# iPieter/llmq

Hardware: AMD Instinct MI355X
Metric: output_tokens_per_sec (Tower-Plus-9B continuous-batching serving decode) (higher is better)
Workload: dtype bf16; 1 GPU; model=tower-plus-9b (gemma-2-9b arch, random init), global_batch=512, seq_len=1024, parallelism=dp1, kv_cache_dtype=auto

## Files before the change

### llmq_amd/engine/model_runner.py

```python

from __future__ import annotations

import logging
import time
from typing import Dict, List, Optional, Tuple

import numpy as np
import torch

from llmq_amd import ops
from llmq_amd.engine.config import EngineConfig
from llmq_amd.engine.forward_meta import ChunkGather, DecodeMeta, MixedMeta, PrefillMeta
from llmq_amd.engine.kv_cache import KVCache
from llmq_amd.engine.models.llama import CausalLM
from llmq_amd.engine.scheduler import ScheduledBatch, Sequence

logger = logging.getLogger(__name__)


def _buckets(max_bs: int) -> List[int]:
    sizes = [1, 2, 4, 8, 16, 24, 32, 48, 64, 96, 128, 192, 256, 384, 512]
    out = [b for b in sizes if b < max_bs]
    out.append(max_bs)
    return out


class ModelRunner:
    def __init__(
        self,
        model: CausalLM,
        kv_cache: KVCache,
        config: EngineConfig,
        device: torch.device,
        max_model_len: int,
    ):
        self.model = model
        self.kv_cache = kv_cache
        self.config = config
        self.device = device
        self.max_model_len = max_model_len
        self.block_size = kv_cache.block_size
        self.max_blocks_per_seq = (max_model_len + self.block_size - 1) // self.block_size
        self.use_graphs = (
            config.enable_hipgraph
            and not config.enforce_eager
            and device.type == "cuda"
        )
        self._graphs: Dict[int, torch.cuda.CUDAGraph] = {}
        self._graph_pool = None
        self.sampling_generator = torch.Generator(device=device if device.type == "cuda" else "cpu")
        self.sampling_generator.manual_seed(config.seed)
        self._sample_step = 0
        self._sample_bufs: Dict[str, Dict[str, torch.Tensor]] = {}
        if self.use_graphs:
            self._alloc_static_buffers()


    def _alloc_static_buffers(self) -> None:
        B = min(self.config.max_num_seqs, self.config.hipgraph_max_batch)
        dev = self.device
        self.graph_max_bs = B
        self.in_ids = torch.zeros(B, dtype=torch.long, device=dev)
        self.in_pos = torch.zeros(B, dtype=torch.long, device=dev)
        self.in_slots = torch.zeros(B, dtype=torch.long, device=dev)
        self.in_block_tables = torch.zeros(
            B, self.max_blocks_per_seq, dtype=torch.int32, device=dev
        )
        self.in_context_lens = torch.ones(B, dtype=torch.int32, device=dev)
        self.out_hidden = torch.zeros(
            B, self.model.spec.hidden_size, dtype=self.model.dtype, device=dev
        )
        self.h_ids = torch.zeros(B, dtype=torch.long, pin_memory=True)
        self.h_pos = torch.zeros(B, dtype=torch.long, pin_memory=True)
        self.h_slots = torch.zeros(B, dtype=torch.long, pin_memory=True)
        self.h_block_tables = torch.zeros(
            B, self.max_blocks_per_seq, dtype=torch.int32, pin_memory=True
        )
        self.h_context_lens = torch.ones(B, dtype=torch.int32, pin_memory=True)
        self._staged_rows: List[Tuple[int, int, int]] = [(-1, -1, 0)] * B

    def capture_graphs(self) -> None:
        if not self.use_graphs:
            return
        t0 = time.perf_counter()
        torch.cuda.synchronize()
        for bs in reversed(_buckets(self.graph_max_bs)):
            meta = DecodeMeta(
                block_tables=self.in_block_tables[:bs],
                context_lens=self.in_context_lens[:bs],
                slot_mapping=self.in_slots[:bs],
            )
            out = self.model.forward(self.in_ids[:bs], self.in_pos[:bs], self.kv_cache, meta)
            torch.cuda.synchronize()
            graph = torch.cuda.CUDAGraph()
            with torch.cuda.graph(graph, pool=self._graph_pool):
                out = self.model.forward(
                    self.in_ids[:bs], self.in_pos[:bs], self.kv_cache, meta
                )
                self.out_hidden[:bs].copy_(out)
            if self._graph_pool is None:
                self._graph_pool = graph.pool()
            self._graphs[bs] = graph
        torch.cuda.synchronize()
        logger.info(
            "captured %d decode hipGraphs (max_bs=%d) in %.1fs",
            len(self._graphs), self.graph_max_bs, time.perf_counter() - t0,
# ... 22 lines not shown
        krow = 0
        for seq, (start, end) in zip(pseqs, chunks):
            n = end - start
            ids.extend(seq.token_ids[start:end])
            pos.extend(range(start, end))
            bt = seq.block_table
            slots.extend(bt[p // bs] * bs + (p % bs) for p in range(start, end))
            if end == seq.num_tokens:
                rel_last.append(cu[-1] + n - 1)
            cu.append(cu[-1] + n)
            if any_chunk:
                for p in range(start):
                    g_blocks.append(bt[p // bs])
                    g_offs.append(p % bs)
                    past_dst.append(krow)
                    krow += 1
                for i in range(cu[-2], cu[-1]):
                    fresh_dst.append(krow)
                    krow += 1
            cu_k.append(cu_k[-1] + end)
        slot_mapping = torch.tensor(slots, dtype=torch.long, device=dev)
        gather = None
        if any_chunk:
            gather = ChunkGather(
                cu_seqlens_k=torch.tensor(cu_k, dtype=torch.int32, device=dev),
                blocks=torch.tensor(g_blocks, dtype=torch.long, device=dev),
                offs=torch.tensor(g_offs, dtype=torch.long, device=dev),
                past_dst=torch.tensor(past_dst, dtype=torch.long, device=dev),
                fresh_dst=torch.tensor(fresh_dst, dtype=torch.long, device=dev),
                total_k=krow,
            )
        meta = PrefillMeta(
            cu_seqlens=torch.tensor(cu, dtype=torch.int32, device=dev),
            max_seqlen=max(e - st for (st, e) in chunks),
            slot_mapping=slot_mapping,
            gather=gather,
        )
        return ids, pos, slot_mapping, meta, rel_last

    @torch.no_grad()
    def execute_prefill(self, seqs: List[Sequence], chunks=None, buf_name: str = "main") -> torch.Tensor:
        if chunks is None:
            chunks = [(0, s.num_tokens) for s in seqs]
        dev = self.device
        ids, pos, slot_mapping, meta, rel_last = self._build_prefill_meta(
            seqs, chunks, dev
        )
        input_ids = torch.tensor(ids, dtype=torch.long, device=dev)
        positions = torch.tensor(pos, dtype=torch.long, device=dev)
        hidden = self.model.forward(input_ids, positions, self.kv_cache, meta)
        if not rel_last:
            return torch.empty(0, dtype=torch.long, device=dev)
        last_hidden = hidden[torch.tensor(rel_last, dtype=torch.long, device=dev)]
        logits = self.model.compute_logits(last_hidden)
        sample_seqs = [s for s, (st, e) in zip(seqs, chunks) if e == s.num_tokens]
        return self._sample(logits, sample_seqs, buf_name)


    @torch.no_grad()
    def execute_mixed(self, batch: "ScheduledBatch") -> torch.Tensor:
        dev = self.device
        dseqs = batch.seqs[: batch.n_decode]
        pseqs = batch.seqs[batch.n_decode :]
        chunks = batch.chunks or [(0, s.num_tokens) for s in pseqs]
        bs = self.block_size
        nd = len(dseqs)

        ids = [s.token_ids[-1] for s in dseqs]
        pos = [s.num_tokens - 1 for s in dseqs]
        slots = [s.block_table[p // bs] * bs + (p % bs) for s, p in zip(dseqs, pos)]
        ctx = [s.num_tokens for s in dseqs]
        p_ids, p_pos, p_slots, pmeta, rel_last = self._build_prefill_meta(
            pseqs, chunks, dev
        )
        ids.extend(p_ids)
        pos.extend(p_pos)

        block_tables = torch.zeros(
            nd, max(len(s.block_table) for s in dseqs), dtype=torch.int32, device=dev
        )
        bt_np = np.zeros(tuple(block_tables.shape), dtype=np.int32)
        for i, s in enumerate(dseqs):
            bt_np[i, : len(s.block_table)] = s.block_table
        block_tables.copy_(torch.from_numpy(bt_np))
        d_slots = torch.tensor(slots, dtype=torch.long, device=dev)
        slot_mapping = torch.cat([d_slots, p_slots])
        meta = MixedMeta(
            n_decode=nd,
            decode=DecodeMeta(
                block_tables=block_tables,
                context_lens=torch.tensor(ctx, dtype=torch.int32, device=dev),
                slot_mapping=d_slots,
            ),
            prefill=pmeta,
            slot_mapping=slot_mapping,
        )
        input_ids = torch.tensor(ids, dtype=torch.long, device=dev)
        positions = torch.tensor(pos, dtype=torch.long, device=dev)
        hidden = self.model.forward(input_ids, positions, self.kv_cache, meta)
        last_idx = list(range(nd)) + [nd + r for r in rel_last]
        last_hidden = hidden[torch.tensor(last_idx, dtype=torch.long, device=dev)]
        logits = self.model.compute_logits(last_hidden)
        sample_seqs = list(dseqs) + [
            s for s, (st, e) in zip(pseqs, chunks) if e == s.num_tokens
        ]
        return self._sample(logits, sample_seqs)


    @torch.no_grad()
    def execute_decode(self, seqs: List[Sequence], force_eager: bool = False) -> torch.Tensor:
        dev = self.device
        B = len(seqs)
        bs = self.block_size
        ids = [s.token_ids[-1] for s in seqs]
        pos = [s.num_tokens - 1 for s in seqs]
        slots = [s.block_table[p // bs] * bs + (p % bs) for s, p in zip(seqs, pos)]
        ctx = [s.num_tokens for s in seqs]

        bucket = self._bucket_for(B) if (self.use_graphs and not force_eager) else None
        if bucket is not None and bucket in self._graphs:
            return self._decode_with_graph(seqs, bucket, ids, pos, slots, ctx)

        block_tables = torch.zeros(
            B, max(len(s.block_table) for s in seqs), dtype=torch.int32, device=dev
        )
        bt_np = np.zeros(tuple(block_tables.shape), dtype=np.int32)
        for i, s in enumerate(seqs):
            bt_np[i, : len(s.block_table)] = s.block_table
        block_tables.copy_(torch.from_numpy(bt_np))
        meta = DecodeMeta(
            block_tables=block_tables,
            context_lens=torch.tensor(ctx, dtype=torch.int32, device=dev),
            slot_mapping=torch.tensor(slots, dtype=torch.long, device=dev),
        )
        input_ids = torch.tensor(ids, dtype=torch.long, device=dev)
        positions = torch.tensor(pos, dtype=torch.long, device=dev)
        hidden = self.model.forward(input_ids, positions, self.kv_cache, meta)
        logits = self.model.compute_logits(hidden)
        return self._sample(logits, seqs)

    def _decode_with_graph(
        self, seqs: List[Sequence], bucket: int, ids, pos, slots, ctx
    ) -> torch.Tensor:
        B = len(seqs)
        self.h_ids[:B] = torch.tensor(ids, dtype=torch.long)
        self.h_pos[:B] = torch.tensor(pos, dtype=torch.long)
        self.h_slots[:B] = torch.tensor(slots, dtype=torch.long)
        self.h_context_lens[:B] = torch.tensor(ctx, dtype=torch.int32)
        self.h_context_lens[B:bucket] = 1
        bt_np = self.h_block_tables.numpy()
        max_w = 1
        for i, s in enumerate(seqs):
            n = len(s.block_table)
            if n > max_w:
                max_w = n
            if self._staged_rows[i] != (s.uid, s.num_preemptions, n):
                bt_np[i, :n] = s.block_table
                self._staged_rows[i] = (s.uid, s.num_preemptions, n)
        if B < bucket:
            self.h_slots[B:bucket] = 0
            self.h_ids[B:bucket] = 0
            self.h_pos[B:bucket] = 0
            for i in range(B, bucket):
                if self._staged_rows[i] != (-1, -1, 0):
                    bt_np[i, :1] = 0
                    self._staged_rows[i] = (-1, -1, 0)
        self.in_ids[:bucket].copy_(self.h_ids[:bucket], non_blocking=True)
        self.in_pos[:bucket].copy_(self.h_pos[:bucket], non_blocking=True)
        self.in_slots[:bucket].copy_(self.h_slots[:bucket], non_blocking=True)
        self.in_context_lens[:bucket].copy_(self.h_context_lens[:bucket], non_blocking=True)
        self.in_block_tables[:bucket, :max_w].copy_(
            self.h_block_tables[:bucket, :max_w], non_blocking=True
        )
        self._graphs[bucket].replay()
        logits = self.model.compute_logits(self.out_hidden[:B])
        return self._sample(logits, seqs)


    def _sample_buf(self, name: str, B: int, dev) -> Dict[str, torch.Tensor]:
        buf = self._sample_bufs.get(name)
        if buf is None or buf["out"].numel() < B:
            cap = max(B, self.config.max_num_seqs)
            buf = {
                "out": torch.empty(cap, dtype=torch.int64, device=dev),
                "keys": torch.empty(cap, dtype=torch.int64, device=dev),
                "temps": torch.empty(cap, dtype=torch.float32, device=dev),
                "temps_h": torch.empty(cap, dtype=torch.float32, pin_memory=True),
                "seeds": torch.empty(cap, dtype=torch.int32, device=dev),
                "seeds_h": torch.empty(cap, dtype=torch.int32, pin_memory=True),
                "pos": torch.empty(cap, dtype=torch.int32, device=dev),
                "pos_h": torch.empty(cap, dtype=torch.int32, pin_memory=True),
            }
            self._sample_bufs[name] = buf
        return buf

    def _sample(self, logits: torch.Tensor, seqs: List[Sequence],
                buf_name: str = "main") -> torch.Tensor:
        dev = logits.device
        self._sample_step += 1
        simple = all(
            s.params.top_k == 0 and s.params.top_p >= 1.0 for s in seqs
        )
        if dev.type == "cuda":
            B = len(seqs)
            buf = self._sample_buf(buf_name, B, dev)
            th = buf["temps_h"]
            sh = buf["seeds_h"]
            ph = buf["pos_h"]
            for i, s in enumerate(seqs):
                th[i] = s.params.temperature
                rs = s.params.seed
                if rs is None:
                    sh[i] = 0
                else:
                    v = rs & 0x7FFFFFFF
                    sh[i] = v if v else 0x1E3779B9
                ph[i] = s.output_len
            buf["temps"][:B].copy_(th[:B], non_blocking=True)
            buf["seeds"][:B].copy_(sh[:B], non_blocking=True)
            buf["pos"][:B].copy_(ph[:B], non_blocking=True)
            logits_f = logits.float()
            bounds = None
            if not simple:
                tps = torch.tensor([s.params.top_p for s in seqs],
                                   dtype=torch.float32, device=dev)
                tks = torch.tensor([s.params.top_k for s in seqs],
                                   dtype=torch.int64, device=dev)
                bounds = ops.topk_topp_bound(
                    logits_f, buf["temps"][:B], tps, tks)
            ops.sample_gumbel_argmax(
                buf["out"][:B], buf["keys"][:B], logits_f,
                buf["temps"][:B], buf["seeds"][:B],
                buf["pos"][:B], self.config.seed, self._sample_step, bounds,
            )
            return buf["out"][:B]
        temps = torch.tensor([s.params.temperature for s in seqs], dtype=torch.float32, device=dev)
        tps = torch.tensor([s.params.top_p for s in seqs], dtype=torch.float32, device=dev)
        tks = torch.tensor([s.params.top_k for s in seqs], dtype=torch.int64, device=dev)
        out = ops.sample_tokens(logits, temps, tps, tks, self.sampling_generator)
        seeded = [
            i for i, s in enumerate(seqs)
            if s.params.seed is not None and s.params.temperature > 0
        ]
        if seeded:
            idx = torch.tensor(seeded, dtype=torch.long, device=dev)
            rows = logits[idx].float().cpu()
            temps_c, tps_c, tks_c = temps[idx].cpu(), tps[idx].cpu(), tks[idx].cpu()
            redraw = torch.empty(len(seeded), dtype=out.dtype)
            for j, i in enumerate(seeded):
                s = seqs[i]
                g = torch.Generator(device="cpu")
                g.manual_seed((s.params.seed << 20) ^ s.output_len)
                redraw[j] = ops.sample_tokens(
                    rows[j : j + 1], temps_c[j : j + 1], tps_c[j : j + 1],
                    tks_c[j : j + 1], g,
                )[0]
            out[idx] = redraw.to(out.device)
        return out
```

### llmq_amd/engine/models/llama.py

```python

from __future__ import annotations

import math
import os
from typing import Dict, List, Optional, Union

import torch
import torch.nn.functional as F

from llmq_amd import ops
from llmq_amd.engine.forward_meta import DecodeMeta, MixedMeta, PrefillMeta
from llmq_amd.engine.kv_cache import KVCache
from llmq_amd.engine.model_specs import ModelSpec
from llmq_amd.parallel import get_tp_group


_USE_SKINNY_GEMM = os.environ.get("LLMQ_SKINNY_GEMM", "0") not in ("0", "false", "")


def _proj(x: torch.Tensor, w: torch.Tensor, bias=None) -> torch.Tensor:
    if (_USE_SKINNY_GEMM and x.is_cuda and x.dtype == torch.bfloat16
            and x.shape[0] <= 1024 and w.shape[1] % 64 == 0
            and w.shape[0] % 4 == 0):
        return ops.skinny_gemm(x, w, bias)
# ... 198 lines not shown
                self.rope_cache, meta.slot_mapping,
            )
            window = s.sliding_window if s.layer_uses_sliding_window(i) else 0
            if meta.is_prefill:
                attn = self._prefill_attn(q, k, v, meta, kv_cache, i, window)
            elif meta.is_mixed:
                nd = meta.n_decode
                attn_d = ops.paged_decode_attention(
                    q[:nd], kv_cache.k[i], kv_cache.v[i],
                    meta.decode.block_tables, meta.decode.context_lens,
                    s.scale, s.attn_softcap, window,
                )
                attn_p = self._prefill_attn(
                    q[nd:], k[nd:], v[nd:], meta.prefill, kv_cache, i, window
                )
                attn = torch.cat([attn_d, attn_p], dim=0)
            else:
                attn = ops.paged_decode_attention(
                    q, kv_cache.k[i], kv_cache.v[i], meta.block_tables,
                    meta.context_lens, s.scale, s.attn_softcap, window,
                )
            attn_out = _proj(attn.reshape(T, self.q_size), lw.o)
            if tp is not None:
                attn_out = tp.all_reduce(attn_out)
            if s.post_norms:
                h, residual = ops.norm_add_norm(
                    attn_out, residual, lw.post_attn_norm, lw.pre_mlp_norm,
                    s.rms_eps, self.norm_offset,
                )
            else:
                h, residual = ops.fused_add_rmsnorm(
                    attn_out, residual, lw.pre_mlp_norm, s.rms_eps, self.norm_offset
                )
            gate_up = _proj(h, lw.gate_up)
            act = ops.gelu_tanh_and_mul(gate_up) if s.gelu else ops.silu_and_mul(gate_up)
            mlp_out = _proj(act, lw.down)
            if tp is not None:
                mlp_out = tp.all_reduce(mlp_out)
            w_next = (
                self.layers[i + 1].input_norm if i + 1 < n_layers else self.final_norm
            )
            if s.post_norms:
                h, residual = ops.norm_add_norm(
                    mlp_out, residual, lw.post_mlp_norm, w_next,
                    s.rms_eps, self.norm_offset,
                )
            else:
                h, residual = ops.fused_add_rmsnorm(
                    mlp_out, residual, w_next, s.rms_eps, self.norm_offset
                )
        return h

    @torch.no_grad()
    def compute_logits(self, hidden: torch.Tensor) -> torch.Tensor:
        logits = _proj(hidden, self.lm_head).float()
        cap = self.spec.final_softcap
        if cap and cap > 0:
            logits = torch.tanh(logits / cap) * cap
        return logits
```

### llmq_amd/ops/__init__.py

```python

from __future__ import annotations

import os
from pathlib import Path
from typing import Optional, Tuple

import torch

from llmq_amd.ops import torch_ref

_EXT = None
_EXT_ERROR: Optional[str] = None
_EXT_TRIED = False


def _try_load_extension() -> None:
    global _EXT, _EXT_ERROR, _EXT_TRIED
    if _EXT_TRIED:
        return
    _EXT_TRIED = True
    here = Path(__file__).parent
    override = os.environ.get("LLMQ_OPS_SO")
    if override:
        candidates = [Path(override)]
# ... 154 lines not shown
    cu_seqlens: torch.Tensor,
    max_seqlen: int,
    scale: float,
    softcap: float = 0.0,
    window: int = 0,
    cu_seqlens_k: Optional[torch.Tensor] = None,
) -> torch.Tensor:
    cu_k = cu_seqlens if cu_seqlens_k is None else cu_seqlens_k
    if _use_hip(q):
        out = torch.empty_like(q)
        _EXT.varlen_prefill_attention(
            out, q, k, v, cu_seqlens, cu_k, int(max_seqlen), scale, softcap, window
        )
        return out
    return torch_ref.varlen_prefill_attention(
        q, k, v, cu_seqlens, scale, softcap, window, cu_seqlens_k=cu_k
    )




def skinny_gemm(
    x: torch.Tensor,
    w: torch.Tensor,
    bias: Optional[torch.Tensor] = None,
    splitk: int = 0,
    out: Optional[torch.Tensor] = None,
) -> torch.Tensor:
    M, K = x.shape
    N = w.shape[0]
    if not (x.is_cuda and x.dtype == torch.bfloat16 and K % 64 == 0
            and N % 4 == 0 and has_hip_ext()):
        import torch.nn.functional as F

        return F.linear(x, w, bias)
    if out is None:
        out = torch.empty(M, N, dtype=torch.bfloat16, device=x.device)
    _EXT.skinny_gemm(out, x, w, bias, splitk)
    return out




def sample_gumbel_argmax(
    out: torch.Tensor,
    keys: torch.Tensor,
    logits: torch.Tensor,
    temps: torch.Tensor,
    req_seeds: torch.Tensor,
    req_pos: torch.Tensor,
    seed: int,
    step: int,
    bounds: Optional[torch.Tensor] = None,
) -> None:
    assert _use_hip(logits)
    keys.zero_()
    _EXT.sample_gumbel_argmax(out, keys, logits, temps, req_seeds, req_pos,
                              seed, step, bounds)


def topk_topp_bound(
    logits: torch.Tensor,
    temps: torch.Tensor,
    top_ps: torch.Tensor,
    top_ks: torch.Tensor,
) -> torch.Tensor:
    assert _use_hip(logits)
    out = torch.empty(logits.size(0), dtype=torch.float32, device=logits.device)
    _EXT.topk_topp_bound(out, logits, temps, top_ps, top_ks)
    return out


def sample_tokens(
    logits: torch.Tensor,
    temperatures: torch.Tensor,
    top_ps: torch.Tensor,
    top_ks: torch.Tensor,
    generator: Optional[torch.Generator] = None,
) -> torch.Tensor:
    if logits.is_cuda:
        return _sample_tokens_gpu(logits, temperatures, top_ps, top_ks, generator)
    return torch_ref.sample_tokens(logits, temperatures, top_ps, top_ks, generator)


def _sample_tokens_gpu(
    logits: torch.Tensor,
    temperatures: torch.Tensor,
    top_ps: torch.Tensor,
    top_ks: torch.Tensor,
    generator: Optional[torch.Generator],
) -> torch.Tensor:
    B, V = logits.shape
    greedy = temperatures <= 0
    temps = torch.where(greedy, torch.ones_like(temperatures), temperatures)
    scaled = logits.float() / temps.unsqueeze(1)
    need_topk = bool((top_ks > 0).any()) and bool((top_ks < V).any())
    need_topp = bool((top_ps < 1.0).any())
    if need_topk or need_topp:
        bound = topk_topp_bound(logits.float(), temperatures.float(),
                                top_ps.float(), top_ks)
        scaled = torch.where(logits.float() >= bound.unsqueeze(1), scaled,
                             torch.full_like(scaled, float("-inf")))
    u = torch.rand(B, V, device=logits.device, generator=generator)
    gumbel = -torch.log(-torch.log(u.clamp_min(1e-20)).clamp_min(1e-20))
    sampled = (scaled + gumbel).argmax(dim=-1)
    greedy_choice = logits.argmax(dim=-1)
    return torch.where(greedy, greedy_choice, sampled)
```

### llmq_amd/ops/hip/bindings.cpp

```cpp

#include <ATen/ATen.h>
#include <c10/hip/HIPStream.h>
#include <hip/hip_runtime.h>
#include <torch/library.h>

#include <hip/hip_bf16.h>
#include <hip/hip_fp16.h>


namespace {

#define CHECK_GPU(x) TORCH_CHECK(x.is_cuda(), #x " must be on GPU")
#define CHECK_LASTDIM(x) \
  TORCH_CHECK(x.stride(-1) == 1, #x " innermost dim must be contiguous")

hipStream_t stream() { return c10::hip::getCurrentHIPStream().stream(); }

template <typename F>
void dispatch_dtype(const at::Tensor& t, const char* name, F&& f) {
  switch (t.scalar_type()) {
    case at::kBFloat16:
      f.template operator()<__hip_bfloat16>();
      break;
    case at::kHalf:
// ... 54 lines not shown
                       reinterpret_cast<T*>(residual.data_ptr()),
                       reinterpret_cast<const T*>(weight.data_ptr()), hidden,
                       (float)eps, (float)offset);
  });
}


template <bool GELU>
void act_and_mul(at::Tensor out, at::Tensor in) {
  CHECK_GPU(in);
  CHECK_LASTDIM(in);
  const int d = out.size(-1);
  const long rows = out.numel() / d;
  TORCH_CHECK(in.size(-1) == 2 * d, "in must be [..., 2*d]");
  const long chunks = rows * (d / 8);
  const int grid = std::min<long>((chunks + 255) / 256, 2048);
  dispatch_dtype(in, "act_and_mul", [&]<typename T>() {
    hipLaunchKernelGGL((act_and_mul_kernel<T, GELU>), dim3(grid), dim3(256), 0,
                       stream(), reinterpret_cast<T*>(out.data_ptr()),
                       reinterpret_cast<const T*>(in.data_ptr()), rows, d);
  });
}

void silu_and_mul(at::Tensor out, at::Tensor in) { act_and_mul<false>(out, in); }
void gelu_tanh_and_mul(at::Tensor out, at::Tensor in) { act_and_mul<true>(out, in); }


void rope_inplace(at::Tensor q, at::Tensor k, at::Tensor positions,
                  at::Tensor cos_sin) {
  CHECK_GPU(q);
  CHECK_LASTDIM(q);
  CHECK_LASTDIM(k);
  TORCH_CHECK(q.dim() == 3 && k.dim() == 3, "q/k must be [T, H, D]");
  TORCH_CHECK(cos_sin.scalar_type() == at::kFloat, "cos_sin must be f32");
  const int T_ = q.size(0);
  if (T_ == 0) return;
  const int hq = q.size(1), hk = k.size(1), d = q.size(2);
  TORCH_CHECK(q.stride(1) == d && k.stride(1) == d, "head dim must be packed");
  dispatch_dtype(q, "rope", [&]<typename T>() {
    hipLaunchKernelGGL(rope_kernel<T>, dim3(T_), dim3(256), 0, stream(),
                       reinterpret_cast<T*>(q.data_ptr()),
                       reinterpret_cast<T*>(k.data_ptr()),
                       positions.data_ptr<long>(), cos_sin.data_ptr<float>(),
                       hq, hk, d, q.stride(0), k.stride(0));
  });
}

void norm_add_norm(at::Tensor x, at::Tensor residual, at::Tensor w_post,
                   at::Tensor w_pre, double eps, double offset) {
  CHECK_GPU(x);
  CHECK_LASTDIM(x);
  const int hidden = x.size(-1);
  const long rows = x.numel() / hidden;
  dispatch_dtype(x, "norm_add_norm", [&]<typename T>() {
    hipLaunchKernelGGL(norm_add_norm_kernel<T>, dim3(rows), dim3(256), 0,
                       stream(), reinterpret_cast<T*>(x.data_ptr()),
                       reinterpret_cast<T*>(residual.data_ptr()),
                       reinterpret_cast<const T*>(w_post.data_ptr()),
                       reinterpret_cast<const T*>(w_pre.data_ptr()), hidden,
                       (float)eps, (float)offset);
  });
}


void reshape_and_cache(at::Tensor key, at::Tensor value, at::Tensor k_cache,
                       at::Tensor v_cache, at::Tensor slot_mapping) {
  CHECK_GPU(key);
  CHECK_LASTDIM(key);
  const int T_ = key.size(0);
  if (T_ == 0) return;
  const int kvh = key.size(1), d = key.size(2);
  const int bs = k_cache.size(2);
  TORCH_CHECK(k_cache.is_contiguous() && v_cache.is_contiguous());
  TORCH_CHECK(slot_mapping.scalar_type() == at::kLong);
  const bool fp8_cache = k_cache.scalar_type() == at::kFloat8_e4m3fn;
  dispatch_dtype(key, "reshape_and_cache", [&]<typename T>() {
    dispatch_cache_type<T>(fp8_cache, [&]<typename TC>() {
      hipLaunchKernelGGL((reshape_and_cache_kernel<T, TC>), dim3(T_), dim3(128),
                         0, stream(), reinterpret_cast<const T*>(key.data_ptr()),
                         reinterpret_cast<const T*>(value.data_ptr()),
                         reinterpret_cast<TC*>(k_cache.data_ptr()),
                         reinterpret_cast<TC*>(v_cache.data_ptr()),
                         slot_mapping.data_ptr<long>(), kvh, d, bs,
                         key.stride(0), value.stride(0));
    });
  });
}

void rope_and_cache(at::Tensor q, at::Tensor k, at::Tensor value,
                    at::Tensor k_cache, at::Tensor v_cache,
                    at::Tensor positions, at::Tensor cos_sin,
                    at::Tensor slot_mapping) {
  CHECK_GPU(q);
  CHECK_LASTDIM(q);
  CHECK_LASTDIM(k);
  TORCH_CHECK(q.dim() == 3 && k.dim() == 3, "q/k must be [T, H, D]");
  TORCH_CHECK(cos_sin.scalar_type() == at::kFloat);
  TORCH_CHECK(slot_mapping.scalar_type() == at::kLong);
  const int T_ = q.size(0);
  if (T_ == 0) return;
  const int hq = q.size(1), hk = k.size(1), d = q.size(2);
  const int bs = k_cache.size(2);
  TORCH_CHECK(q.stride(1) == d && k.stride(1) == d, "head dim must be packed");
  const bool fp8_cache = k_cache.scalar_type() == at::kFloat8_e4m3fn;
  dispatch_dtype(q, "rope_and_cache", [&]<typename T>() {
    dispatch_cache_type<T>(fp8_cache, [&]<typename TC>() {
      hipLaunchKernelGGL((rope_and_cache_kernel<T, TC>), dim3(T_), dim3(256), 0,
                         stream(), reinterpret_cast<T*>(q.data_ptr()),
                         reinterpret_cast<T*>(k.data_ptr()),
                         reinterpret_cast<const T*>(value.data_ptr()),
                         reinterpret_cast<TC*>(k_cache.data_ptr()),
                         reinterpret_cast<TC*>(v_cache.data_ptr()),
                         positions.data_ptr<long>(), cos_sin.data_ptr<float>(),
// ... 189 lines not shown
  TORCH_CHECK(out.scalar_type() == at::kBFloat16 && out.is_contiguous());
  const int M = x.size(0), K = x.size(1), N = w.size(0);
  TORCH_CHECK(w.size(1) == K && out.size(0) == M && out.size(1) == N);
  TORCH_CHECK(K % SKG_BK == 0, "K must be a multiple of 64");
  TORCH_CHECK(N % 4 == 0, "N must be a multiple of 4");
  const __hip_bfloat16* bias_ptr = nullptr;
  if (bias.has_value() && bias->defined()) {
    TORCH_CHECK(bias->scalar_type() == at::kBFloat16 && bias->numel() == N);
    bias_ptr = reinterpret_cast<const __hip_bfloat16*>(bias->data_ptr());
  }
  const int mt = (M + SKG_BM - 1) / SKG_BM;
  const int nt = (N + SKG_BN - 1) / SKG_BN;
  int z = (int)splitk;
  if (z <= 0) {
    z = 1;
    while (mt * nt * z < 256 && (K / SKG_BK) / (z * 2) >= 8 && z < 8) z *= 2;
  }
  dim3 grid(mt, nt, z);
  static const int sync_dbg = [] {
    const char* e = getenv("LLMQ_SKG_SYNC");
    return e ? atoi(e) : 0;
  }();
  if (z == 1) {
    if (sync_dbg) {
      hipLaunchKernelGGL((skinny_gemm_kernel<0, 1>), grid, dim3(SKG_NT), 0,
                         stream(), out.data_ptr(),
                         reinterpret_cast<const __hip_bfloat16*>(x.data_ptr()),
                         reinterpret_cast<const __hip_bfloat16*>(w.data_ptr()),
                         bias_ptr, M, N, K, x.stride(0), w.stride(0));
      return;
    }
    hipLaunchKernelGGL((skinny_gemm_kernel<0>), grid, dim3(SKG_NT), 0, stream(),
                       out.data_ptr(),
                       reinterpret_cast<const __hip_bfloat16*>(x.data_ptr()),
                       reinterpret_cast<const __hip_bfloat16*>(w.data_ptr()),
                       bias_ptr, M, N, K, x.stride(0), w.stride(0));
    return;
  }
  at::Tensor slabs = at::empty({z, (long)M * N}, x.options().dtype(at::kFloat));
  hipLaunchKernelGGL((skinny_gemm_kernel<1>), grid, dim3(SKG_NT), 0, stream(),
                     slabs.data_ptr(),
                     reinterpret_cast<const __hip_bfloat16*>(x.data_ptr()),
                     reinterpret_cast<const __hip_bfloat16*>(w.data_ptr()),
                     nullptr, M, N, K, x.stride(0), w.stride(0));
  const long MN = (long)M * N;
  const long blocks = (MN / 4 + 255) / 256;
  hipLaunchKernelGGL(skinny_gemm_reduce_kernel, dim3(blocks), dim3(256), 0,
                     stream(),
                     reinterpret_cast<__hip_bfloat16*>(out.data_ptr()),
                     slabs.data_ptr<float>(), bias_ptr, z, MN, N);
}


void topk_topp_bound(at::Tensor out_bound, at::Tensor logits, at::Tensor temps,
                     at::Tensor top_ps, at::Tensor top_ks) {
  CHECK_GPU(logits);
  TORCH_CHECK(logits.scalar_type() == at::kFloat && logits.dim() == 2);
  TORCH_CHECK(out_bound.scalar_type() == at::kFloat);
  TORCH_CHECK(top_ps.scalar_type() == at::kFloat);
  TORCH_CHECK(top_ks.scalar_type() == at::kLong);
  const int B = logits.size(0), V = logits.size(1);
  hipLaunchKernelGGL(topk_topp_bound_kernel, dim3(B), dim3(256), 0, stream(),
                     out_bound.data_ptr<float>(), logits.data_ptr<float>(),
                     temps.data_ptr<float>(), top_ps.data_ptr<float>(),
                     top_ks.data_ptr<long>(), V, logits.stride(0));
}

void sample_gumbel_argmax(at::Tensor out, at::Tensor keys, at::Tensor logits,
                          at::Tensor temps, at::Tensor req_seeds,
                          at::Tensor req_pos, long seed, long step,
                          c10::optional<at::Tensor> bounds) {
  CHECK_GPU(logits);
  TORCH_CHECK(logits.scalar_type() == at::kFloat && logits.dim() == 2);
  TORCH_CHECK(out.scalar_type() == at::kLong);
  TORCH_CHECK(keys.scalar_type() == at::kLong && keys.numel() == logits.size(0));
  TORCH_CHECK(req_seeds.scalar_type() == at::kInt);
  TORCH_CHECK(req_pos.scalar_type() == at::kInt);
  const int B = logits.size(0), V = logits.size(1);
  const float* bounds_ptr = nullptr;
  if (bounds.has_value() && bounds->defined()) {
    TORCH_CHECK(bounds->scalar_type() == at::kFloat && bounds->numel() == B);
    bounds_ptr = bounds->data_ptr<float>();
  }
  int nsplit = 1;
  while (B * nsplit < 2048 && nsplit < 64 && (V / nsplit) > 4096) nsplit *= 2;
  hipLaunchKernelGGL(sample_argmax_kernel, dim3(B, nsplit), dim3(256), 0,
                     stream(),
                     reinterpret_cast<unsigned long long*>(keys.data_ptr()),
                     logits.data_ptr<float>(), temps.data_ptr<float>(),
                     reinterpret_cast<const unsigned int*>(req_seeds.data_ptr()),
                     reinterpret_cast<const unsigned int*>(req_pos.data_ptr()),
                     bounds_ptr, V, (unsigned int)seed, (unsigned int)step);
  hipLaunchKernelGGL(unpack_keys_kernel, dim3((B + 255) / 256), dim3(256), 0,
                     stream(), out.data_ptr<long>(),
                     reinterpret_cast<const unsigned long long*>(keys.data_ptr()),
                     B);
}

}

TORCH_LIBRARY(llmq_amd, m) {
  m.def("rmsnorm(Tensor(a!) out, Tensor input, Tensor weight, float eps, float offset) -> ()");
  m.def("fused_add_rmsnorm(Tensor(a!) x, Tensor(b!) residual, Tensor weight, float eps, float offset) -> ()");
  m.def("silu_and_mul(Tensor(a!) out, Tensor input) -> ()");
  m.def("gelu_tanh_and_mul(Tensor(a!) out, Tensor input) -> ()");
  m.def("rope_inplace(Tensor(a!) q, Tensor(b!) k, Tensor positions, Tensor cos_sin) -> ()");
  m.def("reshape_and_cache(Tensor key, Tensor value, Tensor(a!) k_cache, Tensor(b!) v_cache, Tensor slot_mapping) -> ()");
  m.def("paged_decode_attention(Tensor(a!) out, Tensor q, Tensor k_cache, Tensor v_cache, Tensor block_tables, Tensor context_lens, float scale, float softcap, int window) -> ()");
  m.def("varlen_prefill_attention(Tensor(a!) out, Tensor q, Tensor k, Tensor v, Tensor cu_seqlens, Tensor cu_seqlens_k, int max_seqlen, float scale, float softcap, int window) -> ()");
  m.def("sample_gumbel_argmax(Tensor(a!) out, Tensor(b!) keys, Tensor logits, Tensor temps, Tensor req_seeds, Tensor req_pos, int seed, int step, Tensor? bounds=None) -> ()");
  m.def("topk_topp_bound(Tensor(a!) out_bound, Tensor logits, Tensor temps, Tensor top_ps, Tensor top_ks) -> ()");
  m.def("skinny_gemm(Tensor(a!) out, Tensor x, Tensor w, Tensor? bias, int splitk) -> ()");
  m.def("norm_add_norm(Tensor(a!) x, Tensor(b!) residual, Tensor w_post, Tensor w_pre, float eps, float offset) -> ()");
  m.def("rope_and_cache(Tensor(a!) q, Tensor(b!) k, Tensor value, Tensor(c!) k_cache, Tensor(d!) v_cache, Tensor positions, Tensor cos_sin, Tensor slot_mapping) -> ()");
}

TORCH_LIBRARY_IMPL(llmq_amd, CUDA, m) {
  m.impl("rmsnorm", &rmsnorm);
  m.impl("fused_add_rmsnorm", &fused_add_rmsnorm);
  m.impl("silu_and_mul", &silu_and_mul);
  m.impl("gelu_tanh_and_mul", &gelu_tanh_and_mul);
  m.impl("rope_inplace", &rope_inplace);
  m.impl("reshape_and_cache", &reshape_and_cache);
  m.impl("paged_decode_attention", &paged_decode_attention);
  m.impl("varlen_prefill_attention", &varlen_prefill_attention);
  m.impl("sample_gumbel_argmax", &sample_gumbel_argmax);
  m.impl("topk_topp_bound", &topk_topp_bound);
  m.impl("skinny_gemm", &skinny_gemm);
  m.impl("norm_add_norm", &norm_add_norm);
  m.impl("rope_and_cache", &rope_and_cache);
}
```

### llmq_amd/ops/hip/elementwise.hip

```cpp

#include "common.h"


template <typename T>
__global__ void rmsnorm_kernel(T* __restrict__ out, const T* __restrict__ in,
                               const T* __restrict__ weight, int hidden,
                               float eps, float offset) {
  constexpr int VE = Vec8<T>::kElems;
  __shared__ float red[4];
  const int row = blockIdx.x;
  const T* x = in + (long)row * hidden;
  T* o = out + (long)row * hidden;

  float ss = 0.f;
  for (int i = threadIdx.x * VE; i < hidden; i += blockDim.x * VE) {
    Vec8<T> v = load16(x + i);
#pragma unroll
    for (int j = 0; j < VE; ++j) {
      float f = to_f32(v.data[j]);
      ss += f * f;
    }
  }
  ss = block_reduce_sum(ss, red);
  const float inv = rsqrtf(ss / hidden + eps);
// ... 105 lines not shown
}

template <typename T>
__global__ void norm_add_norm_kernel(T* __restrict__ x, T* __restrict__ residual,
                                     const T* __restrict__ w_post,
                                     const T* __restrict__ w_pre, int hidden,
                                     float eps, float offset) {
  constexpr int VE = Vec8<T>::kElems;
  __shared__ float red[4];
  const int row = blockIdx.x;
  T* xr = x + (long)row * hidden;
  T* rr = residual + (long)row * hidden;

  float ss = 0.f;
  for (int i = threadIdx.x * VE; i < hidden; i += blockDim.x * VE) {
    Vec8<T> v = load16(xr + i);
#pragma unroll
    for (int j = 0; j < VE; ++j) {
      float f = to_f32(v.data[j]);
      ss += f * f;
    }
  }
  ss = block_reduce_sum(ss, red);
  const float inv1 = rsqrtf(ss / hidden + eps);

  float ss2 = 0.f;
  for (int i = threadIdx.x * VE; i < hidden; i += blockDim.x * VE) {
    Vec8<T> vx = load16(xr + i);
    Vec8<T> vr = load16(rr + i);
    Vec8<T> vw = load16(w_post + i);
    Vec8<T> nr;
#pragma unroll
    for (int j = 0; j < VE; ++j) {
      const float t = to_f32(vx.data[j]) * inv1 * (to_f32(vw.data[j]) + offset);
      const float r = to_f32(vr.data[j]) + t;
      nr.data[j] = from_f32<T>(r);
      ss2 += r * r;
    }
    store16(rr + i, nr);
  }
  ss2 = block_reduce_sum(ss2, red);
  const float inv2 = rsqrtf(ss2 / hidden + eps);

  for (int i = threadIdx.x * VE; i < hidden; i += blockDim.x * VE) {
    Vec8<T> vr = load16(rr + i);
    Vec8<T> vw = load16(w_pre + i);
    Vec8<T> o;
#pragma unroll
    for (int j = 0; j < VE; ++j)
      o.data[j] = from_f32<T>(to_f32(vr.data[j]) * inv2 * (to_f32(vw.data[j]) + offset));
    store16(xr + i, o);
  }
}
```

### llmq_amd/ops/hip/sampling.hip

```cpp

#include "common.h"

DEVINL unsigned int hash_u32(unsigned int x) {
  x ^= x >> 16; x *= 0x7feb352dU;
  x ^= x >> 15; x *= 0x846ca68bU;
  x ^= x >> 16;
  return x;
}

DEVINL float uniform01(unsigned int seed, unsigned int step, unsigned int b,
                       unsigned int v) {
  unsigned int key = b * 0x9E3779B9u ^ v * 0x85EBCA6Bu ^ step * 0xC2B2AE35u ^ seed;
  unsigned int h = hash_u32(hash_u32(key));
  return (h + 1u) * (1.0f / 4294967296.0f);
}

DEVINL unsigned long long pack_key(float val, int idx) {
  unsigned int u = __float_as_uint(val);
  u = (u & 0x80000000u) ? ~u : (u | 0x80000000u);
  return ((unsigned long long)u << 32) | (unsigned int)(~idx);
}

__global__ __launch_bounds__(256) void sample_argmax_kernel(
    unsigned long long* __restrict__ out_keys,
    const float* __restrict__ logits,
    const float* __restrict__ temps,
    const unsigned int* __restrict__ req_seeds,
    const unsigned int* __restrict__ req_pos,
    const float* __restrict__ bounds,
    int V, unsigned int seed, unsigned int step) {
  const int b = blockIdx.x;
  const int nsplit = gridDim.y;
  const int chunk = (V + nsplit - 1) / nsplit;
  const int v0 = blockIdx.y * chunk;
  const int v1 = min(v0 + chunk, V);
  const float temp = temps[b];
  const bool greedy = temp <= 0.f;
  const float inv_t = greedy ? 1.0f : 1.0f / temp;
  const float* row = logits + (long)b * V;
  const unsigned int rs = req_seeds[b];
  const unsigned int kseed = rs ? rs : seed;
  const unsigned int kstep = rs ? req_pos[b] : step;
  const unsigned int kb = rs ? 0u : (unsigned int)b;
  const float bound = bounds ? bounds[b] : -3e38f;

  float best = -3e38f;
  int best_i = v0;
  for (int v = v0 + threadIdx.x; v < v1; v += 256) {
    if (row[v] < bound) continue;
    float x = row[v] * inv_t;
    if (!greedy) {
      const float u = uniform01(kseed, kstep, kb, v);
      x += -__logf(-__logf(u));
    }
    if (x > best) { best = x; best_i = v; }
  }
  for (int off = WAVE / 2; off > 0; off >>= 1) {
    const float ov = __shfl_xor(best, off, WAVE);
    const int oi = __shfl_xor(best_i, off, WAVE);
    if (ov > best || (ov == best && oi < best_i)) { best = ov; best_i = oi; }
  }
  __shared__ float vals[4];
  __shared__ int idxs[4];
  const int wid = threadIdx.x / WAVE;
  if ((threadIdx.x & (WAVE - 1)) == 0) { vals[wid] = best; idxs[wid] = best_i; }
  __syncthreads();
  if (threadIdx.x == 0) {
    for (int w = 1; w < 4; ++w) {
      if (vals[w] > best || (vals[w] == best && idxs[w] < best_i)) {
        best = vals[w]; best_i = idxs[w];
      }
    }
    atomicMax(out_keys + b, pack_key(best, best_i));
  }
}


#define TH_NBINS 512
#define TH_TPB 256
#define TH_XMIN -32.0f

__global__ __launch_bounds__(TH_TPB) void topk_topp_bound_kernel(
    float* __restrict__ out_bound,
    const float* __restrict__ logits,
    const float* __restrict__ temps,
    const float* __restrict__ top_ps,
    const long* __restrict__ top_ks,
    int V, long stride) {
  const int b = blockIdx.x;
  const int tid = threadIdx.x;
  const float T0 = temps[b];
  const float p_lim = top_ps[b];
  const long k_lim = top_ks[b];
  const bool need_p = p_lim < 1.0f;
  const bool need_k = k_lim > 0 && k_lim < V;
  if (T0 <= 0.f || !(need_p || need_k)) {
    if (tid == 0) out_bound[b] = -3e38f;
    return;
  }
  const float inv_t = 1.0f / T0;
  const float* row = logits + (long)b * stride;

  __shared__ float h_sum[TH_NBINS];
  __shared__ int h_cnt[TH_NBINS];
  __shared__ float red[TH_TPB / WAVE];
  __shared__ float sh_state[6];

  float m = -3e38f;
  for (int v = tid; v < V; v += TH_TPB) m = fmaxf(m, row[v]);
  for (int off = WAVE / 2; off > 0; off >>= 1)
    m = fmaxf(m, __shfl_xor(m, off, WAVE));
  if ((tid & (WAVE - 1)) == 0) red[tid / WAVE] = m;
  __syncthreads();
  if (tid == 0) {
    for (int w = 1; w < TH_TPB / WAVE; ++w) m = fmaxf(m, red[w]);
    red[0] = m;
  }
  __syncthreads();
  m = red[0];

  float xlo = TH_XMIN, xhi = 0.0f;
  float keep_above = 3e38f;
  float p_above = 0.f;
  long n_above = 0;
  float Z = 0.f;
  float bound_x = TH_XMIN;
  bool done = false;

  for (int iter = 0; iter < 2 && !done; ++iter) {
    for (int i = tid; i < TH_NBINS; i += TH_TPB) { h_sum[i] = 0.f; h_cnt[i] = 0; }
    __syncthreads();
    const float w = (xhi - xlo) / TH_NBINS;
    const float inv_w = 1.0f / w;
    float tail = 0.f;
    for (int v = tid; v < V; v += TH_TPB) {
      const float x = (row[v] - m) * inv_t;
      if (x >= keep_above) continue;
      if (x < xlo) { if (iter == 0) tail += __expf(fmaxf(x, -80.f)); continue; }
      int bin = (int)((x - xlo) * inv_w);
      bin = bin < 0 ? 0 : (bin >= TH_NBINS ? TH_NBINS - 1 : bin);
      atomicAdd(&h_sum[bin], __expf(x));
      atomicAdd(&h_cnt[bin], 1);
    }
    for (int off = WAVE / 2; off > 0; off >>= 1) tail += __shfl_xor(tail, off, WAVE);
    if ((tid & (WAVE - 1)) == 0) red[tid / WAVE] = tail;
    __syncthreads();
    if (tid == 0) {
      if (iter == 0) {
        Z = red[0] + red[1] + red[2] + red[3];
        for (int i = 0; i < TH_NBINS; ++i) Z += h_sum[i];
        sh_state[3] = Z;
      } else {
        Z = sh_state[3];
      }
      const float p_target = need_p ? p_lim * Z : 3e38f;
      const long k_target = need_k ? k_lim : 0x7fffffffffffffffL;
      float cum = p_above;
      long cnt = n_above;
      int cross = -1;
      for (int i = TH_NBINS - 1; i >= 0; --i) {
        cum += h_sum[i];
        cnt += h_cnt[i];
        if (cum >= p_target || cnt >= k_target) { cross = i; break; }
      }
      if (cross < 0) {
        sh_state[0] = (iter == 0) ? -3e38f : xlo;
        sh_state[1] = 1.0f;
      } else {
        float pa = p_above;
        long na = n_above;
        for (int i = TH_NBINS - 1; i > cross; --i) { pa += h_sum[i]; na += h_cnt[i]; }
        sh_state[0] = xlo + cross * w;
        sh_state[1] = 0.0f;
        sh_state[2] = xlo + (cross + 1) * w;
        sh_state[4] = (cross == TH_NBINS - 1) ? keep_above
                                              : (xlo + (cross + 1) * w);
        red[0] = pa;
        red[1] = (float)na;
      }
    }
    __syncthreads();
    if (sh_state[1] != 0.0f) {
      bound_x = sh_state[0];
      done = true;
    } else {
      xlo = sh_state[0];
      xhi = sh_state[2];
      keep_above = sh_state[4];
      p_above = red[0];
// ... 16 lines not shown
```

Baseline: 11440 tokens/s.

## Fuse logit softcap and fp32 cast into sampling kernels; add register-resident norm sandwich

The sampling path now passes raw bf16 lm_head logits straight to the gumbel-argmax and top-k/top-p kernels. Those kernels apply the final tanh softcap inline with vectorized 16-byte loads, so the separate fp32 cast and softcap elementwise passes over the B×vocab logits tensor are no longer needed. Separately, a norm_add_norm variant keeps each row in registers so x and residual are read once across both RMSNorms. Both paths are on by default through env flags, and the softcap now runs in the inner sampling loop for every vocab element.

```diff
diff --git a/llmq_amd/engine/model_runner.py b/llmq_amd/engine/model_runner.py
--- a/llmq_amd/engine/model_runner.py
+++ b/llmq_amd/engine/model_runner.py
@@ -2,6 +2,7 @@
 from __future__ import annotations
 
 import logging
+import os
 import time
 from typing import Dict, List, Optional, Tuple
 
@@ -52,6 +53,8 @@
         self.sampling_generator.manual_seed(config.seed)
         self._sample_step = 0
         self._sample_bufs: Dict[str, Dict[str, torch.Tensor]] = {}
+        self.fused_logit_tail = device.type == "cuda" and os.environ.get(
+            "LLMQ_FUSED_LOGIT_TAIL", "1") not in ("0", "false", "")
         if self.use_graphs:
             self._alloc_static_buffers()
 
@@ -180,9 +183,9 @@
         if not rel_last:
             return torch.empty(0, dtype=torch.long, device=dev)
         last_hidden = hidden[torch.tensor(rel_last, dtype=torch.long, device=dev)]
-        logits = self.model.compute_logits(last_hidden)
+        logits, cap = self._logits_for_sampling(last_hidden)
         sample_seqs = [s for s, (st, e) in zip(seqs, chunks) if e == s.num_tokens]
-        return self._sample(logits, sample_seqs, buf_name)
+        return self._sample(logits, sample_seqs, buf_name, softcap=cap)
 
 
     @torch.no_grad()
@@ -228,11 +231,11 @@
         hidden = self.model.forward(input_ids, positions, self.kv_cache, meta)
         last_idx = list(range(nd)) + [nd + r for r in rel_last]
         last_hidden = hidden[torch.tensor(last_idx, dtype=torch.long, device=dev)]
-        logits = self.model.compute_logits(last_hidden)
+        logits, cap = self._logits_for_sampling(last_hidden)
         sample_seqs = list(dseqs) + [
             s for s, (st, e) in zip(pseqs, chunks) if e == s.num_tokens
         ]
-        return self._sample(logits, sample_seqs)
+        return self._sample(logits, sample_seqs, softcap=cap)
 
 
     @torch.no_grad()
@@ -264,8 +267,8 @@
         input_ids = torch.tensor(ids, dtype=torch.long, device=dev)
         positions = torch.tensor(pos, dtype=torch.long, device=dev)
         hidden = self.model.forward(input_ids, positions, self.kv_cache, meta)
-        logits = self.model.compute_logits(hidden)
-        return self._sample(logits, seqs)
+        logits, cap = self._logits_for_sampling(hidden)
+        return self._sample(logits, seqs, softcap=cap)
 
     def _decode_with_graph(
         self, seqs: List[Sequence], bucket: int, ids, pos, slots, ctx
@@ -301,8 +304,8 @@
             self.h_block_tables[:bucket, :max_w], non_blocking=True
         )
         self._graphs[bucket].replay()
-        logits = self.model.compute_logits(self.out_hidden[:B])
-        return self._sample(logits, seqs)
+        logits, cap = self._logits_for_sampling(self.out_hidden[:B])
+        return self._sample(logits, seqs, softcap=cap)
 
 
     def _sample_buf(self, name: str, B: int, dev) -> Dict[str, torch.Tensor]:
@@ -322,8 +325,14 @@
             self._sample_bufs[name] = buf
         return buf
 
+    def _logits_for_sampling(self, hidden: torch.Tensor) -> Tuple[torch.Tensor, float]:
+        if self.fused_logit_tail:
+            cap = self.model.spec.final_softcap
+            return self.model.lm_head_logits(hidden), float(cap) if cap and cap > 0 else 0.0
+        return self.model.compute_logits(hidden), 0.0
+
     def _sample(self, logits: torch.Tensor, seqs: List[Sequence],
-                buf_name: str = "main") -> torch.Tensor:
+                buf_name: str = "main", softcap: float = 0.0) -> torch.Tensor:
         dev = logits.device
         self._sample_step += 1
         simple = all(
@@ -347,7 +356,7 @@
             buf["temps"][:B].copy_(th[:B], non_blocking=True)
             buf["seeds"][:B].copy_(sh[:B], non_blocking=True)
             buf["pos"][:B].copy_(ph[:B], non_blocking=True)
-            logits_f = logits.float()
+            logits_f = logits if self.fused_logit_tail else logits.float()
             bounds = None
             if not simple:
                 tps = torch.tensor([s.params.top_p for s in seqs],
@@ -355,11 +364,12 @@
                 tks = torch.tensor([s.params.top_k for s in seqs],
                                    dtype=torch.int64, device=dev)
                 bounds = ops.topk_topp_bound(
-                    logits_f, buf["temps"][:B], tps, tks)
+                    logits_f, buf["temps"][:B], tps, tks, softcap)
             ops.sample_gumbel_argmax(
                 buf["out"][:B], buf["keys"][:B], logits_f,
                 buf["temps"][:B], buf["seeds"][:B],
                 buf["pos"][:B], self.config.seed, self._sample_step, bounds,
+                softcap,
             )
             return buf["out"][:B]
         temps = torch.tensor([s.params.temperature for s in seqs], dtype=torch.float32, device=dev)
diff --git a/llmq_amd/engine/models/llama.py b/llmq_amd/engine/models/llama.py
--- a/llmq_amd/engine/models/llama.py
+++ b/llmq_amd/engine/models/llama.py
@@ -274,6 +274,10 @@
         return h
 
     @torch.no_grad()
+    def lm_head_logits(self, hidden: torch.Tensor) -> torch.Tensor:
+        return _proj(hidden, self.lm_head)
+
+    @torch.no_grad()
     def compute_logits(self, hidden: torch.Tensor) -> torch.Tensor:
         logits = _proj(hidden, self.lm_head).float()
         cap = self.spec.final_softcap
diff --git a/llmq_amd/ops/__init__.py b/llmq_amd/ops/__init__.py
--- a/llmq_amd/ops/__init__.py
+++ b/llmq_amd/ops/__init__.py
@@ -230,11 +230,12 @@
     seed: int,
     step: int,
     bounds: Optional[torch.Tensor] = None,
+    softcap: float = 0.0,
 ) -> None:
     assert _use_hip(logits)
     keys.zero_()
     _EXT.sample_gumbel_argmax(out, keys, logits, temps, req_seeds, req_pos,
-                              seed, step, bounds)
+                              seed, step, bounds, softcap)
 
 
 def topk_topp_bound(
@@ -242,10 +243,11 @@
     temps: torch.Tensor,
     top_ps: torch.Tensor,
     top_ks: torch.Tensor,
+    softcap: float = 0.0,
 ) -> torch.Tensor:
     assert _use_hip(logits)
     out = torch.empty(logits.size(0), dtype=torch.float32, device=logits.device)
-    _EXT.topk_topp_bound(out, logits, temps, top_ps, top_ks)
+    _EXT.topk_topp_bound(out, logits, temps, top_ps, top_ks, softcap)
     return out
 
 
diff --git a/llmq_amd/ops/hip/bindings.cpp b/llmq_amd/ops/hip/bindings.cpp
--- a/llmq_amd/ops/hip/bindings.cpp
+++ b/llmq_amd/ops/hip/bindings.cpp
@@ -130,13 +130,27 @@
   CHECK_LASTDIM(x);
   const int hidden = x.size(-1);
   const long rows = x.numel() / hidden;
+  const char* re = getenv("LLMQ_NORM_SANDWICH_REGS");
+  const bool regs = (!re || atoi(re) != 0) && x.element_size() == 2 &&
+                    hidden % 8 == 0 && hidden <= 8192;
   dispatch_dtype(x, "norm_add_norm", [&]<typename T>() {
-    hipLaunchKernelGGL(norm_add_norm_kernel<T>, dim3(rows), dim3(256), 0,
-                       stream(), reinterpret_cast<T*>(x.data_ptr()),
-                       reinterpret_cast<T*>(residual.data_ptr()),
-                       reinterpret_cast<const T*>(w_post.data_ptr()),
-                       reinterpret_cast<const T*>(w_pre.data_ptr()), hidden,
-                       (float)eps, (float)offset);
+    auto launch = [&](void (*kernel)(T*, T*, const T*, const T*, int, float,
+                                     float)) {
+      hipLaunchKernelGGL(kernel, dim3(rows), dim3(256), 0, stream(),
+                         reinterpret_cast<T*>(x.data_ptr()),
+                         reinterpret_cast<T*>(residual.data_ptr()),
+                         reinterpret_cast<const T*>(w_post.data_ptr()),
+                         reinterpret_cast<const T*>(w_pre.data_ptr()), hidden,
+                         (float)eps, (float)offset);
+    };
+    if constexpr (sizeof(T) == 2) {
+      if (regs) {
+        launch(hidden <= 4096 ? norm_add_norm_regs_kernel<T, 2>
+                              : norm_add_norm_regs_kernel<T, 4>);
+        return;
+      }
+    }
+    launch(norm_add_norm_kernel<T>);
   });
 }
 
@@ -432,26 +446,39 @@
 }
 
 
+float softcap_reciprocal(double softcap) {
+  return softcap > 0 ? 1.0f / (float)softcap : 0.0f;
+}
+
 void topk_topp_bound(at::Tensor out_bound, at::Tensor logits, at::Tensor temps,
-                     at::Tensor top_ps, at::Tensor top_ks) {
+                     at::Tensor top_ps, at::Tensor top_ks, double softcap) {
   CHECK_GPU(logits);
-  TORCH_CHECK(logits.scalar_type() == at::kFloat && logits.dim() == 2);
+  CHECK_LASTDIM(logits);
+  TORCH_CHECK(logits.dim() == 2);
   TORCH_CHECK(out_bound.scalar_type() == at::kFloat);
+  TORCH_CHECK(temps.scalar_type() == at::kFloat);
   TORCH_CHECK(top_ps.scalar_type() == at::kFloat);
   TORCH_CHECK(top_ks.scalar_type() == at::kLong);
   const int B = logits.size(0), V = logits.size(1);
-  hipLaunchKernelGGL(topk_topp_bound_kernel, dim3(B), dim3(256), 0, stream(),
-                     out_bound.data_ptr<float>(), logits.data_ptr<float>(),
-                     temps.data_ptr<float>(), top_ps.data_ptr<float>(),
-                     top_ks.data_ptr<long>(), V, logits.stride(0));
+  if (B == 0) return;
+  dispatch_dtype(logits, "topk_topp_bound", [&]<typename T>() {
+    hipLaunchKernelGGL(topk_topp_bound_kernel<T>, dim3(B), dim3(256), 0,
+                       stream(), out_bound.data_ptr<float>(),
+                       reinterpret_cast<const T*>(logits.data_ptr()),
+                       temps.data_ptr<float>(), top_ps.data_ptr<float>(),
+                       top_ks.data_ptr<long>(), V, logits.stride(0),
+                       (float)softcap, softcap_reciprocal(softcap));
+  });
 }
 
 void sample_gumbel_argmax(at::Tensor out, at::Tensor keys, at::Tensor logits,
                           at::Tensor temps, at::Tensor req_seeds,
                           at::Tensor req_pos, long seed, long step,
-                          c10::optional<at::Tensor> bounds) {
+                          c10::optional<at::Tensor> bounds, double softcap) {
   CHECK_GPU(logits);
-  TORCH_CHECK(logits.scalar_type() == at::kFloat && logits.dim() == 2);
+  CHECK_LASTDIM(logits);
+  TORCH_CHECK(logits.dim() == 2);
+  TORCH_CHECK(temps.scalar_type() == at::kFloat);
   TORCH_CHECK(out.scalar_type() == at::kLong);
   TORCH_CHECK(keys.scalar_type() == at::kLong && keys.numel() == logits.size(0));
   TORCH_CHECK(req_seeds.scalar_type() == at::kInt);
@@ -464,13 +491,17 @@
   }
   int nsplit = 1;
   while (B * nsplit < 2048 && nsplit < 64 && (V / nsplit) > 4096) nsplit *= 2;
-  hipLaunchKernelGGL(sample_argmax_kernel, dim3(B, nsplit), dim3(256), 0,
-                     stream(),
-                     reinterpret_cast<unsigned long long*>(keys.data_ptr()),
-                     logits.data_ptr<float>(), temps.data_ptr<float>(),
-                     reinterpret_cast<const unsigned int*>(req_seeds.data_ptr()),
-                     reinterpret_cast<const unsigned int*>(req_pos.data_ptr()),
-                     bounds_ptr, V, (unsigned int)seed, (unsigned int)step);
+  const int chunk = ((V + nsplit - 1) / nsplit + 7) / 8 * 8;
+  dispatch_dtype(logits, "sample_gumbel_argmax", [&]<typename T>() {
+    hipLaunchKernelGGL(
+        sample_argmax_kernel<T>, dim3(B, nsplit), dim3(256), 0, stream(),
+        reinterpret_cast<unsigned long long*>(keys.data_ptr()),
+        reinterpret_cast<const T*>(logits.data_ptr()), temps.data_ptr<float>(),
+        reinterpret_cast<const unsigned int*>(req_seeds.data_ptr()),
+        reinterpret_cast<const unsigned int*>(req_pos.data_ptr()), bounds_ptr,
+        V, logits.stride(0), chunk, (float)softcap,
+        softcap_reciprocal(softcap), (unsigned int)seed, (unsigned int)step);
+  });
   hipLaunchKernelGGL(unpack_keys_kernel, dim3((B + 255) / 256), dim3(256), 0,
                      stream(), out.data_ptr<long>(),
                      reinterpret_cast<const unsigned long long*>(keys.data_ptr()),
@@ -488,8 +519,8 @@
   m.def("reshape_and_cache(Tensor key, Tensor value, Tensor(a!) k_cache, Tensor(b!) v_cache, Tensor slot_mapping) -> ()");
   m.def("paged_decode_attention(Tensor(a!) out, Tensor q, Tensor k_cache, Tensor v_cache, Tensor block_tables, Tensor context_lens, float scale, float softcap, int window) -> ()");
   m.def("varlen_prefill_attention(Tensor(a!) out, Tensor q, Tensor k, Tensor v, Tensor cu_seqlens, Tensor cu_seqlens_k, int max_seqlen, float scale, float softcap, int window) -> ()");
-  m.def("sample_gumbel_argmax(Tensor(a!) out, Tensor(b!) keys, Tensor logits, Tensor temps, Tensor req_seeds, Tensor req_pos, int seed, int step, Tensor? bounds=None) -> ()");
-  m.def("topk_topp_bound(Tensor(a!) out_bound, Tensor logits, Tensor temps, Tensor top_ps, Tensor top_ks) -> ()");
+  m.def("sample_gumbel_argmax(Tensor(a!) out, Tensor(b!) keys, Tensor logits, Tensor temps, Tensor req_seeds, Tensor req_pos, int seed, int step, Tensor? bounds=None, float softcap=0.0) -> ()");
+  m.def("topk_topp_bound(Tensor(a!) out_bound, Tensor logits, Tensor temps, Tensor top_ps, Tensor top_ks, float softcap=0.0) -> ()");
   m.def("skinny_gemm(Tensor(a!) out, Tensor x, Tensor w, Tensor? bias, int splitk) -> ()");
   m.def("norm_add_norm(Tensor(a!) x, Tensor(b!) residual, Tensor w_post, Tensor w_pre, float eps, float offset) -> ()");
   m.def("rope_and_cache(Tensor(a!) q, Tensor(b!) k, Tensor value, Tensor(c!) k_cache, Tensor(d!) v_cache, Tensor positions, Tensor cos_sin, Tensor slot_mapping) -> ()");
diff --git a/llmq_amd/ops/hip/elementwise.hip b/llmq_amd/ops/hip/elementwise.hip
--- a/llmq_amd/ops/hip/elementwise.hip
+++ b/llmq_amd/ops/hip/elementwise.hip
@@ -181,3 +181,71 @@
     store16(xr + i, o);
   }
 }
+
+template <typename T, int NV>
+__global__ __launch_bounds__(256) void norm_add_norm_regs_kernel(
+    T* __restrict__ x, T* __restrict__ residual, const T* __restrict__ w_post,
+    const T* __restrict__ w_pre, int hidden, float eps, float offset) {
+  constexpr int VE = Vec8<T>::kElems;
+  __shared__ float red[4];
+  const int row = blockIdx.x;
+  T* xr = x + (long)row * hidden;
+  T* rr = residual + (long)row * hidden;
+
+  Vec8<T> vx[NV], vr[NV], vwp[NV], vwn[NV];
+#pragma unroll
+  for (int k = 0; k < NV; ++k) {
+    const int i = threadIdx.x * VE + k * 256 * VE;
+    if (i < hidden) {
+      vx[k] = load16(xr + i);
+      vr[k] = load16(rr + i);
+      vwp[k] = load16(w_post + i);
+      vwn[k] = load16(w_pre + i);
+    }
+  }
+
+  float ss = 0.f;
+#pragma unroll
+  for (int k = 0; k < NV; ++k) {
+    const int i = threadIdx.x * VE + k * 256 * VE;
+    if (i < hidden) {
+#pragma unroll
+      for (int j = 0; j < VE; ++j) {
+        float f = to_f32(vx[k].data[j]);
+        ss += f * f;
+      }
+    }
+  }
+  ss = block_reduce_sum(ss, red);
+  const float inv1 = rsqrtf(ss / hidden + eps);
+
+  float ss2 = 0.f;
+#pragma unroll
+  for (int k = 0; k < NV; ++k) {
+    const int i = threadIdx.x * VE + k * 256 * VE;
+    if (i < hidden) {
+#pragma unroll
+      for (int j = 0; j < VE; ++j) {
+        const float t = to_f32(vx[k].data[j]) * inv1 * (to_f32(vwp[k].data[j]) + offset);
+        const float r = to_f32(vr[k].data[j]) + t;
+        vr[k].data[j] = from_f32<T>(r);
+        ss2 += r * r;
+      }
+      store16(rr + i, vr[k]);
+    }
+  }
+  ss2 = block_reduce_sum(ss2, red);
+  const float inv2 = rsqrtf(ss2 / hidden + eps);
+
+#pragma unroll
+  for (int k = 0; k < NV; ++k) {
+    const int i = threadIdx.x * VE + k * 256 * VE;
+    if (i < hidden) {
+      Vec8<T> o;
+#pragma unroll
+      for (int j = 0; j < VE; ++j)
+        o.data[j] = from_f32<T>(to_f32(vr[k].data[j]) * inv2 * (to_f32(vwn[k].data[j]) + offset));
+      store16(xr + i, o);
+    }
+  }
+}
diff --git a/llmq_amd/ops/hip/sampling.hip b/llmq_amd/ops/hip/sampling.hip
--- a/llmq_amd/ops/hip/sampling.hip
+++ b/llmq_amd/ops/hip/sampling.hip
@@ -21,23 +21,37 @@
   return ((unsigned long long)u << 32) | (unsigned int)(~idx);
 }
 
+template <typename T>
+DEVINL float logit_value(T raw, float softcap, float inv_cap) {
+#pragma clang fp contract(off)
+  float x = to_f32(raw);
+  if (softcap > 0.f) {
+    x = x * inv_cap;
+    x = tanhf(x);
+    x = x * softcap;
+  }
+  return x;
+}
+
+template <typename T>
 __global__ __launch_bounds__(256) void sample_argmax_kernel(
     unsigned long long* __restrict__ out_keys,
-    const float* __restrict__ logits,
+    const T* __restrict__ logits,
     const float* __restrict__ temps,
     const unsigned int* __restrict__ req_seeds,
     const unsigned int* __restrict__ req_pos,
     const float* __restrict__ bounds,
-    int V, unsigned int seed, unsigned int step) {
+    int V, long stride, int chunk, float softcap, float inv_cap,
+    unsigned int seed, unsigned int step) {
+  constexpr int VE = Vec8<T>::kElems;
   const int b = blockIdx.x;
-  const int nsplit = gridDim.y;
-  const int chunk = (V + nsplit - 1) / nsplit;
   const int v0 = blockIdx.y * chunk;
+  if (v0 >= V) return;
   const int v1 = min(v0 + chunk, V);
   const float temp = temps[b];
   const bool greedy = temp <= 0.f;
   const float inv_t = greedy ? 1.0f : 1.0f / temp;
-  const float* row = logits + (long)b * V;
+  const T* row = logits + (long)b * stride;
   const unsigned int rs = req_seeds[b];
   const unsigned int kseed = rs ? rs : seed;
   const unsigned int kstep = rs ? req_pos[b] : step;
@@ -46,15 +60,26 @@
 
   float best = -3e38f;
   int best_i = v0;
-  for (int v = v0 + threadIdx.x; v < v1; v += 256) {
-    if (row[v] < bound) continue;
-    float x = row[v] * inv_t;
+  auto consider = [&](int v, T raw) {
+    const float l = logit_value(raw, softcap, inv_cap);
+    if (l < bound) return;
+    float x = l * inv_t;
     if (!greedy) {
       const float u = uniform01(kseed, kstep, kb, v);
       x += -__logf(-__logf(u));
     }
     if (x > best) { best = x; best_i = v; }
-  }
+  };
+  const int mis = (int)(((unsigned long)(row + v0) / sizeof(T)) % VE);
+  const int vb = min(v1, v0 + (mis ? VE - mis : 0));
+  const int ve = vb + (v1 - vb) / VE * VE;
+  if (v0 + (int)threadIdx.x < vb) consider(v0 + threadIdx.x, row[v0 + threadIdx.x]);
+  for (int v = vb + threadIdx.x * VE; v < ve; v += 256 * VE) {
+    const Vec8<T> vec = load16(row + v);
+#pragma unroll
+    for (int j = 0; j < VE; ++j) consider(v + j, vec.data[j]);
+  }
+  if (ve + (int)threadIdx.x < v1) consider(ve + threadIdx.x, row[ve + threadIdx.x]);
   for (int off = WAVE / 2; off > 0; off >>= 1) {
     const float ov = __shfl_xor(best, off, WAVE);
     const int oi = __shfl_xor(best_i, off, WAVE);
@@ -80,13 +105,14 @@
 #define TH_TPB 256
 #define TH_XMIN -32.0f
 
+template <typename T>
 __global__ __launch_bounds__(TH_TPB) void topk_topp_bound_kernel(
     float* __restrict__ out_bound,
-    const float* __restrict__ logits,
+    const T* __restrict__ logits,
     const float* __restrict__ temps,
     const float* __restrict__ top_ps,
     const long* __restrict__ top_ks,
-    int V, long stride) {
+    int V, long stride, float softcap, float inv_cap) {
   const int b = blockIdx.x;
   const int tid = threadIdx.x;
   const float T0 = temps[b];
@@ -99,7 +125,7 @@
     return;
   }
   const float inv_t = 1.0f / T0;
-  const float* row = logits + (long)b * stride;
+  const T* row = logits + (long)b * stride;
 
   __shared__ float h_sum[TH_NBINS];
   __shared__ int h_cnt[TH_NBINS];
@@ -107,7 +133,8 @@
   __shared__ float sh_state[6];
 
   float m = -3e38f;
-  for (int v = tid; v < V; v += TH_TPB) m = fmaxf(m, row[v]);
+  for (int v = tid; v < V; v += TH_TPB)
+    m = fmaxf(m, logit_value(row[v], softcap, inv_cap));
   for (int off = WAVE / 2; off > 0; off >>= 1)
     m = fmaxf(m, __shfl_xor(m, off, WAVE));
   if ((tid & (WAVE - 1)) == 0) red[tid / WAVE] = m;
@@ -134,7 +161,7 @@
     const float inv_w = 1.0f / w;
     float tail = 0.f;
     for (int v = tid; v < V; v += TH_TPB) {
-      const float x = (row[v] - m) * inv_t;
+      const float x = (logit_value(row[v], softcap, inv_cap) - m) * inv_t;
       if (x >= keep_above) continue;
       if (x < xlo) { if (iter == 0) tail += __expf(fmaxf(x, -80.f)); continue; }
       int bin = (int)((x - xlo) * inv_w);
```

Result: faster. 11630 tokens/s (median of 6 runs) (+1.7%).
